# QData/ChromeGCN

Hardware: AMD Instinct MI355X
Metric: GCN windows/sec (2-layer, d_model=128) on GM12878 Hi-C graph (higher is better)
Workload: dtype f32

## Files before the change

### chromegcn_amd/_lib.py

```python
import ctypes
import os

import torch

from . import _build

_c_int = ctypes.c_int
_c_vp = ctypes.c_void_p
_c_sz = ctypes.c_size_t
_c_float = ctypes.c_float
_c_uint = ctypes.c_uint

_TYPES = {"i": _c_int, "u": _c_uint, "ll": ctypes.c_longlong, "z": _c_sz, "f": _c_float, "zp": ctypes.POINTER(_c_sz)}
_HEADER = {
    "cgcn_abi_version": (_c_int, ""),
    "cgcn_strerror": (ctypes.c_char_p, "code:i"),
    "cgcn_spmm": (_c_int, "stream n_rows:i n_cols:i S:i d:i rowptr col val row_scale X Y aux"),
    "cgcn_layer_fwd": (_c_int, "stream n:i S:i d:i rowptr col val row_scale X W b wg cg Xn Z H gate dropout_p:f rng_state "
                               "stream_id:u H_in colstats colstats_rows:i aux"),
    "cgcn_layer_fwd_colstats_plan": (_c_int, "n:i S:i d:i mode:i rows_per_tile"),
    "cgcn_debug_set_fwd_split_bytes": (None, "bytes:ll"),
    "cgcn_debug_set_products": (None, "mode:i"),
    "cgcn_debug_get_products": (_c_int, ""),
    "cgcn_debug_layer_fwd_route": (_c_int, "n:i S:i d:i aux colstats_rows:i"),
    "cgcn_debug_layer_bwd_route": (_c_int, "n:i S:i d:i"),
    "cgcn_layer_bwd_workspace_bytes": (_c_sz, "n:i S:i d:i"),
    "cgcn_layer_bwd": (_c_int, "stream n:i S:i d:i rowptr_t col_t val_t row_scale X Z H gate W wg dXn dgate dX dHs dW db dwg "
                               "dcg accumulate:i in_dropout_p:f rng_state in_stream_id:u head workspace workspace_bytes:z "
                               "aux_stream sgd aux_t"),
    "cgcn_debug_layer_bwd_phases": (_c_int, "stream n:i S:i d:i rowptr_t col_t val_t row_scale X Z H gate W wg dXn dgate dX dHs "
                                            "dW db dwg dcg accumulate:i in_dropout_p:f rng_state in_stream_id:u head workspace "
                                            "workspace_bytes:z phases:i aux_t"),
    "cgcn_layer_bwd_co": (_c_int, "stream n:i S:i d:i rowptr_t col_t val_t row_scale X Z H gate W wg dXn dgate dX dHs dW db "
                                  "dwg dcg accumulate:i in_dropout_p:f rng_state in_stream_id:u head workspace "
                                  "workspace_bytes:z aux_stream sgd aux_t companion"),
    "cgcn_debug_layer_bwd_co_route": (_c_int, "n:i S:i d:i rowptr_t col_t val_t have_dX:i aux_t companion"),
    "cgcn_head_workspace_bytes": (_c_sz, "n:i S:i d:i C:i"),
    "cgcn_head_workspace_layout": (_c_int, "n:i S:i d:i C:i dym_offset:zp bnc_offset:zp part_offset:zp"),
    "cgcn_head_bwd_partials": (_c_int, "n:i"),
    "cgcn_head_fwd": (_c_int, "stream n:i S:i d:i C:i X bn_w bn_b run_mean run_var num_batches_tracked momentum:f eps:f "
                              "training:i W_out b_out target dropout_p:f rng_state probs loss dpred save_mean save_invstd "
                              "workspace workspace_bytes:z"),
    "cgcn_head_logits": (_c_int, "stream n:i S:i d:i C:i X bn_w bn_b run_mean run_var eps:f W_out b_out logits"),
    "cgcn_head_train": (_c_int, "stream n:i S:i d:i C:i X bn_w bn_b run_mean run_var num_batches_tracked momentum:f eps:f "
                                "W_out b_out target dropout_p:f rng_state probs loss save_mean save_invstd col_stats "
                                "col_stats_tiles:i col_stats_rows:i workspace workspace_bytes:z"),
    "cgcn_debug_head_train_phases": (_c_int, "stream n:i S:i d:i C:i X bn_w bn_b run_mean run_var num_batches_tracked "
                                             "momentum:f eps:f W_out b_out target dropout_p:f rng_state probs loss save_mean "
                                             "save_invstd col_stats col_stats_tiles:i col_stats_rows:i workspace "
                                             "workspace_bytes:z phases:i"),
    "cgcn_head_bwd": (_c_int, "stream n:i S:i d:i C:i X bn_w bn_b save_mean save_invstd W_out dpred dloss dropout_p:f "
                              "rng_state dX dW_out db_out dbn_w dbn_b accumulate:i workspace workspace_bytes:z"),
    "cgcn_sddmm": (_c_int, "stream n:i S:i d:i rowptr col A B out accumulate:i"),
    "cgcn_saliency_normalize": (_c_int, "stream n:i rowptr val raw out"),
    "cgcn_graph_count": (_c_int, "stream n:i adj_type:i rowptr_in col_in val_in row_counts rowptr_out"),
    "cgcn_graph_fill": (_c_int, "stream n:i adj_type:i rowptr_in col_in val_in rowptr_out col_out val_out row_scale "
                                "symmetric_flag"),
    "cgcn_metrics_workspace_bytes": (_c_sz, "n:ll C:i"),
    "cgcn_multilabel_metrics": (_c_int, "stream n:ll C:i probs targets fdr_cutoff:f out workspace workspace_bytes:z"),
    "cgcn_multilabel_metrics_nonneg": (_c_int, "stream n:ll C:i probs targets fdr_cutoff:f out bad workspace "
                                               "workspace_bytes:z"),
    "cgcn_sgd_step": (_c_int, "stream count:ll param grad momentum_buf lr:f momentum:f weight_decay:f nesterov:i "
                              "grad_scale:f rng_state"),
    "cgcn_adam_step": (_c_int, "stream count:ll param grad exp_avg exp_avg_sq step n_step:i ticket lr:f beta1:f beta2:f "
                               "eps:f weight_decay:f grad_scale:f rng_state"),
    "cgcn_ablation_prepare": (_c_int, "stream n:i C:i targets label_bits pos_lists pos_ranks pos_counts"),
    "cgcn_ablation_workspace_bytes": (_c_sz, "n_inst:i S:i d:i layers:i"),
    "cgcn_ablation_layer": (_c_int, "stream n:i S:i d:i rowptr col val row_scale X X_inst W b wg cg label_bits C:i pos_list "
                                    "pos_rank n_pos:i cols n_cols:i X_out removed"),
    "cgcn_ablation_head": (_c_int, "stream n:i S:i d:i C:i X X_inst bn_w bn_b run_mean run_var eps:f W_out b_out pos_lists "
                                   "pos_counts label:i n_pos:i cols n_cols:i removed base M"),
    "cgcn_ablation_mask": (_c_int, "stream n:i C:i rowptr col val row_scale label_bits label_i:i label_j:i val_out "
                                   "row_scale_out removed"),
    "cgcn_ablation_reduce": (_c_int, "stream n:i S:i C:i logits pos_lists pos_counts label:i col_label:i removed base M"),
    "cgcn_hic_workspace_bytes": (_c_sz, "M:ll N:i capacity:ll K:ll"),
    "cgcn_hic_count": (_c_int, "stream M:ll pos1 pos2 window_start N:i workspace workspace_bytes:z n_survivors"),
    "cgcn_hic_build": (_c_int, "stream M:ll pos1 pos2 count norm n_bins:ll resolution_bp:i window_start N:i K:ll capacity:ll "
                               "workspace workspace_bytes:z rowptr_out col_out nnz_out n_survivors"),
    "cgcn_hic_up_workspace_bytes": (_c_sz, "M:ll N:i capacity:ll K:ll resolution_bp:i window_bp:i n_window_bins:ll"),
    "cgcn_hic_count_up": (_c_int, "stream M:ll pos1 pos2 window_start N:i resolution_bp:i window_bp:i n_window_bins:ll workspace "
                                  "workspace_bytes:z n_survivors"),
    "cgcn_hic_build_up": (_c_int, "stream M:ll pos1 pos2 count norm n_bins:ll resolution_bp:i window_bp:i n_window_bins:ll "
                                  "window_start N:i K:ll capacity:ll workspace workspace_bytes:z rowptr_out col_out nnz_out "
                                  "n_survivors"),
    "cgcn_hic_count_dist": (_c_int, "stream M:ll pos1 pos2 window_start N:i min_distance_bp:ll workspace workspace_bytes:z "
                                    "n_survivors"),
    "cgcn_hic_build_dist": (_c_int, "stream M:ll pos1 pos2 count norm n_bins:ll resolution_bp:i window_start N:i K:ll "
                                    "capacity:ll min_distance_bp:ll expected n_expected:ll workspace workspace_bytes:z rowptr_out "
                                    "col_out nnz_out n_survivors"),
    "cgcn_hic_count_up_dist": (_c_int, "stream M:ll pos1 pos2 window_start N:i resolution_bp:i window_bp:i n_window_bins:ll "
                                       "min_distance_bp:ll workspace workspace_bytes:z n_survivors"),
    "cgcn_hic_build_up_dist": (_c_int, "stream M:ll pos1 pos2 count norm n_bins:ll resolution_bp:i window_bp:i n_window_bins:ll "
                                       "window_start N:i K:ll capacity:ll min_distance_bp:ll expected n_expected:ll workspace "
                                       "workspace_bytes:z rowptr_out col_out nnz_out n_survivors"),
    "cgcn_hicdist_workspace_bytes": (_c_sz, "M:ll n_bins:ll"),
    "cgcn_hicdist_sums": (_c_int, "stream M:ll pos1 pos2 count norm n_norm:ll resolution_bp:i n_bins:ll workspace "
                                  "workspace_bytes:z raw_out act_out sizes"),
    "cgcn_text_workspace_bytes": (_c_sz, "n_bytes:ll"),
    "cgcn_text_count": (_c_int, "stream text n_bytes:ll workspace workspace_bytes:z n_records"),
    "cgcn_text_parse": (_c_int, "stream text n_bytes:ll M:ll pos1_out pos2_out count_out flags flag_capacity:ll flag_totals "
                                "workspace workspace_bytes:z"),
    "cgcn_tsne_workspace_bytes": (_c_sz, "n:i"),
    "cgcn_tsne_sqdist": (_c_int, "stream n:i d:i ld:i X D"),
    "cgcn_tsne_affinities": (_c_int, "stream n:i ld:i D perplexity:f C beta"),
    "cgcn_tsne_symmetrize": (_c_int, "stream n:i ld:i C P workspace workspace_bytes:z"),
    "cgcn_tsne_gradient": (_c_int, "stream n:i ld:i P Y exaggeration:f grad want_kl:i workspace workspace_bytes:z"),
# ... 187 lines not shown
```

### chromegcn_amd/csrc/cgcn_head.hip

```cpp
#include "cgcn_common.hpp"

#define HEAD_STAT_BLOCKS 128
#define HEAD_TILE 16
#define HEADB_TILE 32
#ifndef HEAD_MAX_PARTIALS
#define HEAD_MAX_PARTIALS 256
#endif


template <int D>
__global__ __launch_bounds__(256) void k_head_colstats(int n, int S, int rows_per_blk, const float* __restrict__ X,
                                                       float* __restrict__ part) {
  constexpr int RL = 256 / D;
  __shared__ float sm[2][256];
  const int c = threadIdx.x % D, rl = threadIdx.x / D;
  const int r0 = blockIdx.x * rows_per_blk, r1 = min(n, r0 + rows_per_blk);
  for (int s = 0; s < S; ++s) {
    const float* Xs = X + (size_t)s * n * D + c;
    const float pivot = r0 < n ? fmaxf(Xs[(size_t)r0 * D], 0.f) : 0.f;
    float s1 = 0.f, s2 = 0.f;
    int i = r0 + rl;
    for (; i + 3 * RL < r1; i += 4 * RL) {
      float v[4];
#pragma unroll
      for (int u = 0; u < 4; ++u) v[u] = Xs[(size_t)(i + u * RL) * D];
#pragma unroll
      for (int u = 0; u < 4; ++u) {
        const float dlt = fmaxf(v[u], 0.f) - pivot;
        s1 += dlt;
        s2 += dlt * dlt;
      }
    }
    for (; i < r1; i += RL) {
      const float dlt = fmaxf(Xs[(size_t)i * D], 0.f) - pivot;
      s1 += dlt;
      s2 += dlt * dlt;
    }
    if (RL > 1) {
      if (rl > 0) { sm[0][threadIdx.x] = s1; sm[1][threadIdx.x] = s2; }
      __syncthreads();
      if (rl == 0) {
        for (int o = 1; o < RL; ++o) { s1 += sm[0][o * D + c]; s2 += sm[1][o * D + c]; }
      }
      __syncthreads();
    }
    if (rl == 0) {
      const float k = (float)max(r1 - r0, 1);
      float* p = part + (((size_t)blockIdx.x * S + s) * D + c) * 2;
      p[0] = pivot + s1 / k;
      p[1] = fmaxf(s2 - s1 * s1 / k, 0.f);
    }
  }
}

__device__ __forceinline__ void chan_combine_d(double& nA, double& meanA, double& m2A, double nB, double meanB, double m2B) {
  const double nAB = nA + nB;
  if (nAB > 0.0) {
    const double delta = meanB - meanA;
    meanA += delta * (nB / nAB);
    m2A += m2B + delta * delta * (nA * nB / nAB);
    nA = nAB;
  }
}

template <int COLS>
__global__ __launch_bounds__(1024) void k_head_bn_finalize(int n, int S, int D, int nblk, int rows_per_blk,
                                                           const float* __restrict__ part, float momentum, float eps,
                                                           float* __restrict__ run_mean, float* __restrict__ run_var,
                                                           long long* __restrict__ nbt, float* __restrict__ save_mean,
                                                           float* __restrict__ save_invstd) {
  constexpr int NSL = 1024 / COLS;
  constexpr int SPW = 64 / COLS;
  constexpr int NWV = 16;
  static_assert(COLS * SPW == 64 && NSL == SPW * NWV, "thread layout");
  constexpr int KEEP = 16;
  __shared__ double sm[2][NWV][COLS + 1];
  __shared__ double stat[2][COLS + 1];
  const int cl = threadIdx.x % COLS, slice = threadIdx.x / COLS, wave = threadIdx.x >> 6;
  const int CPB = COLS / S;
  const int s = cl / CPB, c = blockIdx.x * CPB + cl % CPB;
  if (blockIdx.x == 0 && threadIdx.x == 0 && nbt) nbt[0] += S;
  float rm = 0.f, rv = 0.f;
// ... 1263 lines not shown
#pragma unroll
              for (int s = 0; s < 2; ++s) {
                float dy = g * invS;
                if (DROP) dy = dropout_keep(key, (uint32_t)((s * n + i) * D + c), thresh) ? dy * keep_scale : 0.f;
                if (s == 1) dy = S2 ? dy : 0.f;
                const float xh = (fmaxf(xq[s][mb][e], 0.f) - mu[s]) * is[s];
                sdy[s] += dy;
                sdyx[s] += dy * xh;
              }
            }
          }
      }
      RS_STAMP(3);
      __syncthreads();
      RS_STAMP(4);
      if (k < mt) load_xq((int)blockIdx.x + k * G);
      if (k >= 1) {
        OPAQUE_LANE(r, q, lq);
        __builtin_amdgcn_s_setprio(0);
        const float* __restrict__ Pa = Pt[(k - 1) & 1] + q * LDP + r;
        const float* __restrict__ Ya = Yt[(k - 1) & 1] + q * LDY + own * 16 + r;
        float a0[NB], a1[NB], b0, b1;
        b0 = Ya[0];
#pragma unroll
        for (int ib = 0; ib < NB; ++ib) a0[ib] = Pa[ib * 16];
#pragma unroll
        for (int kk = 0; kk < TR / 4; kk += 2) {
          b1 = Ya[(kk + 1) * 4 * LDY];
#pragma unroll
          for (int ib = 0; ib < NB; ++ib) a1[ib] = Pa[(kk + 1) * 4 * LDP + ib * 16];
          __builtin_amdgcn_sched_barrier(0);
#pragma unroll
          for (int ib = 0; ib < NB; ++ib) accW[ib] = __builtin_amdgcn_mfma_f32_16x16x4f32(a0[ib], b0, accW[ib], 0, 0, 0);
          __builtin_amdgcn_sched_barrier(0);
          if (kk + 2 < TR / 4) {
            b0 = Ya[(kk + 2) * 4 * LDY];
#pragma unroll
            for (int ib = 0; ib < NB; ++ib) a0[ib] = Pa[(kk + 2) * 4 * LDP + ib * 16];
          }
          __builtin_amdgcn_sched_barrier(0);
#pragma unroll
          for (int ib = 0; ib < NB; ++ib) accW[ib] = __builtin_amdgcn_mfma_f32_16x16x4f32(a1[ib], b1, accW[ib], 0, 0, 0);
          __builtin_amdgcn_sched_barrier(0);
        }
        __builtin_amdgcn_s_setprio(0);
      }
      RS_STAMP(5);
      __syncthreads();
    }
    const int r = lane & 15, q = lane >> 4;
#pragma unroll
    for (int ib = 0; ib < CBMAX; ++ib)
#pragma unroll
      for (int e = 0; e < 4; ++e) {
        const float v = ib < NB ? accW[ib < NB ? ib : 0][e] : 0.f;
        if (c0 + ib * 16 < CPT) P[(size_t)(c0 + ib * 16 + q * 4 + e) * D + own * 16 + r] = v;
      }
    if (last) {
      double* out = (double*)(P + CPT * D + CPT);
#pragma unroll
      for (int s = 0; s < 2; ++s) {
        double a = (double)sdy[s], b = (double)sdyx[s];
        a += __shfl_xor(a, 16); a += __shfl_xor(a, 32);
        b += __shfl_xor(b, 16); b += __shfl_xor(b, 32);
        if (q == 0) {
          out[s * D + own * 16 + r] = a;
          out[(2 + s) * D + own * 16 + r] = b;
          if (sa.acc && s < S) {
            int fa, fb;
            head_bacc_points(wmax, 16, keep_scale, n, fa, fb);
            unsigned long long* bb = bacc_base(sa.acc, S, D);
            bacc_add(bb, S, D, (int)blockIdx.x & (STAT_ACC_SLOTS - 1), s, own * 16 + r, a, b, fa, fb);
            if (blockIdx.x == 0 && s == 0 && own == 0 && r == 0)
              bb[(size_t)STAT_ACC_SLOTS * S * D * 2 + BACC_EXP] = ((unsigned long long)(unsigned)(fb + 1024) << 32) | (unsigned long long)(unsigned)(fa + 1024);
          }
        }
      }
    }
    __syncthreads();
  }
#undef OPAQUE_LANE
}

template <bool MULTI, int NB, bool DROP>
__global__ __launch_bounds__(1024) void k_head_fused_sp(int n, int S, int C, const float* __restrict__ X,
                                                        const float* __restrict__ bn_w, const float* __restrict__ bn_b,
                                                        const float* __restrict__ mean, const float* __restrict__ invstd,
                                                        const float* __restrict__ Wout, const float* __restrict__ bout,
                                                        const float* __restrict__ target, float keep_scale, uint32_t thresh,
                                                        const unsigned long long* __restrict__ rng_state, float inv_count,
                                                        float* __restrict__ probs, float* __restrict__ loss_part,
                                                        float* __restrict__ dym, float* __restrict__ part,
                                                        int c0, int Cp, int CPT, int first_, int last_, HeadStatAcc sa) {
  constexpr int D = 128, TR = 16, EPL = 2, RPW = TR / 8;
  constexpr int LVT = TR * 256;
  constexpr int WLV = 128 * 256;
  __shared__ __attribute__((aligned(16))) unsigned char Wl[3 * WLV];
  __shared__ __attribute__((aligned(16))) unsigned char Ytb[2][3 * LVT];
  __shared__ __attribute__((aligned(16))) unsigned char Ptb[2][3 * LVT];
  __shared__ float lsum[8];
  __shared__ float wmax[16];
  const bool first = MULTI ? first_ != 0 : true, last = MULTI ? last_ != 0 : true;

  const int lane = threadIdx.x & 63;
  const int wave = __builtin_amdgcn_readfirstlane(threadIdx.x >> 6);
  const int own = wave & 7;
  const uint32_t key = DROP ? dropout_key(rng_state, HEAD_STREAM_ID) : 0u;
  const float invS = 1.f / (float)S;
  const bool S2 = S > 1;
  const int PS = head_part_stride(CPT, D);
  const int ntiles = (n + TR - 1) / TR;
  const int G = (int)gridDim.x;
  const int mt = (int)blockIdx.x < ntiles ? (ntiles - 1 - (int)blockIdx.x) / G + 1 : 0;
  float* P = part + (size_t)blockIdx.x * PS;

  float mwl = 0.f;
  for (int idx = threadIdx.x; idx < 128 * (D / 4); idx += 1024) {
    const int j = idx / (D / 4), c4 = idx % (D / 4);
    f32x4 v = (f32x4){0.f, 0.f, 0.f, 0.f};
    if (j < Cp) v = *(const f32x4*)&Wout[(size_t)(c0 + j) * D + c4 * 4];
    u32x2 h2, m2, l2;
    sp_split4(v, h2, m2, l2);
    unsigned char* w = Wl + j * 256 + (((c4 >> 1) ^ sp_sigma(j & 15)) << 4) + ((c4 & 1) << 3);
    *(u32x2*)w = h2;
    *(u32x2*)(w + WLV) = m2;
    *(u32x2*)(w + 2 * WLV) = l2;
    mwl = fmaxf(fmaxf(mwl, fmaxf(fabsf(v[0]), fabsf(v[1]))), fmaxf(fabsf(v[2]), fabsf(v[3])));
  }
  if (sa.acc && last) {
    float mw;
    if (MULTI) mw = head_wout_absmax(Wout, C * (D / 4), 1024);
    else {
      mw = mwl;
#pragma unroll
      for (int o = 32; o > 0; o >>= 1) mw = fmaxf(mw, __shfl_xor(mw, o, WAVE));
    }
    if ((threadIdx.x & 63) == 0) wmax[threadIdx.x >> 6] = mw;
  }
  float* const stash = (float*)Ptb[1];
  static_assert(3 * LVT >= 6 * D * (int)sizeof(float), "the stash fits a P tile");
  if (sa.acc) head_stat_stage<D>(sa, n, S, stash, 1024);
#define OPAQUE_LANE(r_, q_, l_)          \
  int l_ = lane;                         \
  asm volatile("" : "+v"(l_));           \
  const int r_ = l_ & 15, q_ = l_ >> 4

  if (wave < 8) {
    float xv[RPW][2][EPL], tgv[4], mu[2][EPL], is[2][EPL], gw[EPL], gb[EPL];
    float dbo = 0.f, lacc = 0.f;
    const float bj = own * 16 + (lane & 15) < Cp ? bout[c0 + own * 16 + (lane & 15)] : 0.f;
#pragma unroll
    for (int e = 0; e < EPL; ++e) {
      const int c = lane * EPL + e;
      gw[e] = bn_w[c];
      gb[e] = bn_b[c];
    }
    bf16x8 wh[4], wm[4], wl[4];
    {
      const int r = lane & 15, q = lane >> 4;
      const int j = own * 16 + r;
#pragma unroll
      for (int s4 = 0; s4 < 4; ++s4) {
        f32x4 v0 = {0.f, 0.f, 0.f, 0.f}, v1 = v0;
        if (j < Cp) {
          v0 = *(const f32x4*)&Wout[(size_t)(c0 + j) * D + 32 * s4 + 8 * q];
          v1 = *(const f32x4*)&Wout[(size_t)(c0 + j) * D + 32 * s4 + 8 * q + 4];
        }
        const float v[8] = {v0[0], v0[1], v0[2], v0[3], v1[0], v1[1], v1[2], v1[3]};
        sp_split8(v, wh[s4], wm[s4], wl[s4]);
      }
    }
    auto load_rows = [&](int tile) {
      const int node0 = tile * TR;
#pragma unroll
      for (int t = 0; t < RPW; ++t) {
        const int i = node0 + own + t * 8;
#pragma unroll
        for (int s = 0; s < 2; ++s) {
          if (i < n && s < S) ld_row<EPL>(xv[t][s], &X[(unsigned)((s * n + i) * D + lane * EPL)]);
          else zero_row<EPL>(xv[t][s]);
        }
      }
    };
    auto load_targets = [&](int tile) {
      const int node0 = tile * TR;
      const int j = own * 16 + (lane & 15), q = lane >> 4;
#pragma unroll
      for (int e = 0; e < 4; ++e) {
        const int i = node0 + q * 4 + e;
        tgv[e] = (i < n && j < Cp) ? target[(unsigned)(i * C + c0 + j)] : 0.f;
      }
    };
    if (mt > 0) {
      load_rows(blockIdx.x);
      load_targets(blockIdx.x);
    }
    __syncthreads();
#pragma unroll
    for (int e = 0; e < EPL; ++e)
#pragma unroll
      for (int s = 0; s < 2; ++s) head_stat<D>(sa, stash, mean, invstd, s < S ? s : 0, lane * EPL + e, mu[s][e], is[s][e]);
    for (int k = 0; k <= mt; ++k) {
      const int tile = (int)blockIdx.x + k * G;
      const int node0 = tile * TR;
      if (k < mt) {
        int lane_ = lane;
        asm volatile("" : "+v"(lane_));
        unsigned char* __restrict__ Yb = Ytb[k & 1];
#pragma unroll
        for (int t = 0; t < RPW; ++t) {
          const int rr = own + t * 8;
          const int i = node0 + rr;
          float ym[EPL];
#pragma unroll
          for (int e = 0; e < EPL; ++e) {
            float y[2];
#pragma unroll
            for (int s = 0; s < 2; ++s) {
              y[s] = (fmaxf(xv[t][s][e], 0.f) - mu[s][e]) * is[s][e] * gw[e] + gb[e];
              if (DROP) y[s] = dropout_keep(key, (uint32_t)((s * n + i) * D + lane_ * EPL + e), thresh) ? y[s] * keep_scale : 0.f;
            }
            const float a = y[0] + (S2 ? y[1] : 0.f);
            ym[e] = i < n ? a * invS : 0.f;
          }
          uint32_t yh, ymid, yl;
          sp_split2(ym[0], ym[1], yh, ymid, yl);
          unsigned char* w = Yb + rr * 256 + (((lane_ >> 2) ^ sp_sigma(rr)) << 4) + ((lane_ & 3) << 2);
          *(uint32_t*)w = yh;
          *(uint32_t*)(w + LVT) = ymid;
          *(uint32_t*)(w + 2 * LVT) = yl;
        }
      }
      __syncthreads();
      f32x4 acc = {0.f, 0.f, 0.f, 0.f};
      if (k < mt) {
        if (k + 1 < mt) load_rows(tile + G);
        if (own < NB) {
          OPAQUE_LANE(r, q, lq);
          const unsigned char* __restrict__ Ya = Ytb[k & 1] + r * 256 + ((q ^ (sp_sigma(r) & 3)) << 4);
          const int hi = sp_sigma(r) >> 2;
          SpAcc sacc;
          sacc.zero();
#pragma unroll
          for (int s4 = 0; s4 < 4; ++s4) {
            const int o = (s4 ^ hi) << 6;
            const bf16x8 ah = __builtin_bit_cast(bf16x8, *(const u32x4*)(Ya + o));
            const bf16x8 am = __builtin_bit_cast(bf16x8, *(const u32x4*)(Ya + LVT + o));
            const bf16x8 al = __builtin_bit_cast(bf16x8, *(const u32x4*)(Ya + 2 * LVT + o));
            sacc.step(ah, am, al, wh[s4], wm[s4], wl[s4]);
          }
          acc = sacc.sum();
        }
      }
      if (k < mt) {
        unsigned char* __restrict__ Pb = Ptb[k & 1];
        OPAQUE_LANE(r, q, lq);
        const int j = own * 16 + r;
#pragma unroll
        for (int e = 0; e < 4; ++e) {
          const int row = q * 4 + e;
          const int i = node0 + row;
          const bool ok = i < n && j < Cp;
          const float pred = acc[e] + bj;
          const float en = __expf(-fabsf(pred));
          const float inv = __builtin_amdgcn_rcpf(1.f + en);
          const float p = pred >= 0.f ? inv : en * inv;
          const float l = fmaxf(pred, 0.f) - pred * tgv[e] + __logf(1.f + en);
          lacc += ok ? l : 0.f;
          if (ok) probs[(unsigned)(i * C + c0 + j)] = p;
          const float dp = ok ? (p - tgv[e]) * inv_count : 0.f;
          dbo += dp;
          uint16_t dh, dm, dl;
          sp_split1(dp, dh, dm, dl);
          unsigned char* w = Pb + row * 256 + (((j >> 3) ^ sp_sigma(row)) << 4) + ((j & 7) << 1);
          *(uint16_t*)w = dh;
          *(uint16_t*)(w + LVT) = dm;
          *(uint16_t*)(w + 2 * LVT) = dl;
        }
        if (k + 1 < mt) load_targets(tile + G);
      }
      __syncthreads();
    }
    dbo += __shfl_xor(dbo, 16);
    dbo += __shfl_xor(dbo, 32);
    if ((lane >> 4) == 0 && c0 + own * 16 + (lane & 15) < CPT) P[CPT * D + c0 + own * 16 + (lane & 15)] = dbo;
    lacc = wave_sum(lacc);
    if (lane == 0) lsum[own] = lacc;
    __syncthreads();
    if (threadIdx.x == 0) {
      float t = 0.f;
#pragma unroll
      for (int w = 0; w < 8; ++w) t += lsum[w];
      const float tl = first ? t : loss_part[blockIdx.x] + t;
      loss_part[blockIdx.x] = tl;
      if (sa.acc && last) head_loss_ticket(sa, S, D, tl, inv_count);
    }
  } else {
    f32x16 accW[2];
#pragma unroll
    for (int bb = 0; bb < 2; ++bb)
#pragma unroll
      for (int e = 0; e < 16; ++e) accW[bb][e] = 0.f;
    float sdy[2] = {0.f, 0.f}, sdyx[2] = {0.f, 0.f}, mu[2], is[2];
    __syncthreads();
    if (sa.acc && blockIdx.x == 0 && first && wave == 8) head_stat_bookkeeping<D>(sa, stash, S, lane);
#pragma unroll
    for (int s = 0; s < 2; ++s) head_stat<D>(sa, stash, mean, invstd, s < S ? s : 0, own * 16 + (lane & 15), mu[s], is[s]);
    float xq[2][4];
    auto load_xq = [&](int tile) {
      OPAQUE_LANE(r, q, lq);
      const int node0 = tile * TR, c = own * 16 + r;
#pragma unroll
      for (int s = 0; s < 2; ++s)
#pragma unroll
        for (int e = 0; e < 4; ++e) {
          const int i = node0 + q * 4 + e;
          xq[s][e] = (last && i < n && s < S) ? X[(unsigned)((s * n + i) * D + c)] : 0.f;
        }
    };
    for (int k = 0; k <= mt; ++k) {
      const int node0 = ((int)blockIdx.x + (k - 1) * G) * TR;
      f32x4 accY = {0.f, 0.f, 0.f, 0.f};
      if (k >= 1) {
        const unsigned char* __restrict__ Pb = Ptb[(k - 1) & 1];
        OPAQUE_LANE(r, q, lq);
        const unsigned char* __restrict__ Pa = Pb + r * 256 + ((q ^ (sp_sigma(r) & 3)) << 4);
        const int hi = sp_sigma(r) >> 2;
        const int qp = r >> 2, pp = r & 3;
        SpAcc2 sacc;
        sacc.zero();
#pragma unroll
        for (int s4 = 0; s4 < 4; ++s4) {
          const int o = (s4 ^ hi) << 6;
          const bf16x8 ah = __builtin_bit_cast(bf16x8, *(const u32x4*)(Pa + o));
          const bf16x8 am = __builtin_bit_cast(bf16x8, *(const u32x4*)(Pa + LVT + o));
          const bf16x8 al = __builtin_bit_cast(bf16x8, *(const u32x4*)(Pa + 2 * LVT + o));
          int wo[2];
#pragma unroll
          for (int rd = 0; rd < 2; ++rd) {
            const int lrow = 32 * s4 + 8 * q + 4 * rd + qp;
            wo[rd] = lrow * 256 + (((2 * own + (pp >> 1)) ^ sp_sigma(lrow & 15)) << 4) + ((pp & 1) << 3);
          }
          const bf16x8 bh = tr_pair(Wl + wo[0], Wl + wo[1]);
          const bf16x8 bm = tr_pair(Wl + WLV + wo[0], Wl + WLV + wo[1]);
          const bf16x8 bl = tr_pair(Wl + 2 * WLV + wo[0], Wl + 2 * WLV + wo[1]);
          sacc.step(ah, am, al, bh, bm, bl);
        }
        accY = sacc.sum();
        if (MULTI && !first) {
          const int c = own * 16 + r;
#pragma unroll
          for (int e = 0; e < 4; ++e) {
            const int i = node0 + q * 4 + e;
            accY[e] += i < n ? dym[(unsigned)(i * D + c)] : 0.f;
          }
        }
      }
      if (k >= 1) {
        OPAQUE_LANE(r, q, lq);
        const int c = own * 16 + r;
#pragma unroll
        for (int e = 0; e < 4; ++e) {
          const int i = node0 + q * 4 + e;
          const float g = accY[e];
          if (i < n) dym[(unsigned)(i * D + c)] = g;
          if (last) {
#pragma unroll
            for (int s = 0; s < 2; ++s) {
              float dy = g * invS;
              if (DROP) dy = dropout_keep(key, (uint32_t)((s * n + i) * D + c), thresh) ? dy * keep_scale : 0.f;
              if (s == 1) dy = S2 ? dy : 0.f;
              const float xh = (fmaxf(xq[s][e], 0.f) - mu[s]) * is[s];
              sdy[s] += dy;
              sdyx[s] += dy * xh;
            }
          }
        }
      }
      __syncthreads();
      if (k < mt) load_xq((int)blockIdx.x + k * G);
      if (k >= 1) {
        int lq = lane;
        asm volatile("" : "+v"(lq));
        const int hh = lq >> 5, c16 = (lq >> 4) & 1, qp = (lq & 15) >> 2, pp = lq & 3;
        const int cbk = own >> 1, lb0 = 2 * (own & 1);
        const unsigned char* __restrict__ Pb = Ptb[(k - 1) & 1];
        const unsigned char* __restrict__ Yb = Ytb[(k - 1) & 1];
        int ty[2], tp[2];
#pragma unroll
        for (int rd = 0; rd < 2; ++rd) {
          const int row = 8 * hh + 4 * rd + qp, sg = sp_sigma(row);
          ty[rd] = row * 256 + (((4 * cbk + 2 * c16 + (pp >> 1)) ^ sg) << 4) + ((pp & 1) << 3);
          tp[rd] = row * 256 + (((4 * lb0 + 2 * c16 + (pp >> 1)) ^ sg) << 4) + ((pp & 1) << 3);
        }
        bf16x8 yf[3];
#pragma unroll
        for (int v = 0; v < 3; ++v) yf[v] = tr_pair(Yb + v * LVT + ty[0], Yb + v * LVT + ty[1]);
#pragma unroll
        for (int bb = 0; bb < 2; ++bb) {
          bf16x8 pf[3];
#pragma unroll
          for (int v = 0; v < 3; ++v) pf[v] = tr_pair(Pb + v * LVT + (tp[0] ^ (bb << 6)), Pb + v * LVT + (tp[1] ^ (bb << 6)));
          accW[bb] = __builtin_amdgcn_mfma_f32_32x32x16_bf16(pf[2], yf[0], accW[bb], 0, 0, 0);
          accW[bb] = __builtin_amdgcn_mfma_f32_32x32x16_bf16(pf[0], yf[2], accW[bb], 0, 0, 0);
          accW[bb] = __builtin_amdgcn_mfma_f32_32x32x16_bf16(pf[1], yf[1], accW[bb], 0, 0, 0);
          accW[bb] = __builtin_amdgcn_mfma_f32_32x32x16_bf16(pf[1], yf[0], accW[bb], 0, 0, 0);
          accW[bb] = __builtin_amdgcn_mfma_f32_32x32x16_bf16(pf[0], yf[1], accW[bb], 0, 0, 0);
          accW[bb] = __builtin_amdgcn_mfma_f32_32x32x16_bf16(pf[0], yf[0], accW[bb], 0, 0, 0);
        }
      }
      __syncthreads();
    }
    {
      const int hh = lane >> 5, cbk = own >> 1, lb0 = 2 * (own & 1);
#pragma unroll
      for (int bb = 0; bb < 2; ++bb)
#pragma unroll
        for (int e = 0; e < 16; ++e) {
          const int lab = 32 * (lb0 + bb) + (e & 3) + 8 * (e >> 2) + 4 * hh;
          if (c0 + (lab & ~15) < CPT) P[(size_t)(c0 + lab) * D + 32 * cbk + (lane & 31)] = accW[bb][e];
        }
    }
    const int r = lane & 15, q = lane >> 4;
    if (last) {
      double* out = (double*)(P + CPT * D + CPT);
#pragma unroll
      for (int s = 0; s < 2; ++s) {
        double a = (double)sdy[s], b = (double)sdyx[s];
        a += __shfl_xor(a, 16); a += __shfl_xor(a, 32);
        b += __shfl_xor(b, 16); b += __shfl_xor(b, 32);
        if (q == 0) {
          out[s * D + own * 16 + r] = a;
          out[(2 + s) * D + own * 16 + r] = b;
          if (sa.acc && s < S) {
            int fa, fb;
            head_bacc_points(wmax, 16, keep_scale, n, fa, fb);
            unsigned long long* bb = bacc_base(sa.acc, S, D);
            bacc_add(bb, S, D, (int)blockIdx.x & (STAT_ACC_SLOTS - 1), s, own * 16 + r, a, b, fa, fb);
            if (blockIdx.x == 0 && s == 0 && own == 0 && r == 0)
              bb[(size_t)STAT_ACC_SLOTS * S * D * 2 + BACC_EXP] = ((unsigned long long)(unsigned)(fb + 1024) << 32) | (unsigned long long)(unsigned)(fa + 1024);
          }
        }
      }
    }
    __syncthreads();
  }
#undef OPAQUE_LANE
}

__global__ __launch_bounds__(512) void k_head_bwd_finalize(int wslab0, int wslabs, int P, int n, int S, int D, int C, int CP,
                                                           const float* __restrict__ part, float* __restrict__ dWout,
                                                           float* __restrict__ dbout, float* __restrict__ dbn_w,
                                                           float* __restrict__ dbn_b, float* __restrict__ bnc,
                                                           int accumulate, const float* __restrict__ dloss) {
  if ((int)blockIdx.x < wslabs)
    head_finalize_slab<512>(wslab0 + blockIdx.x, P, D, C, CP, part, dWout, dbout, accumulate, dloss);
// ... 99 lines not shown
  return CGCN_OK;
}

int cgcn_head_bwd_partials(int n) { return head_bwd_partials(n); }

size_t cgcn_head_workspace_bytes(int n, int S, int d, int C) {
  if (head_check(n, S, d, C) != CGCN_OK) return 0;
  return 4 * (align4(ws_stats(S, d)) + align4(ws_loss(n)) + align4(ws_dym(n, d)) + align4(ws_bnc(d)) + align4(ws_part(n, d, C)));
}

int cgcn_head_fwd(cgcn_stream_t stream, int n, int S, int d, int C, const float* X, const float* bn_w,
                  const float* bn_b, float* run_mean, float* run_var, long long* num_batches_tracked, float momentum,
                  float eps, int training, const float* Wout, const float* bout, const float* target, float dropout_p,
                  const unsigned long long* rng_state, float* probs, float* loss, float* dpred, float* save_mean,
                  float* save_invstd, void* workspace, size_t workspace_bytes) {
  int rc = head_check(n, S, d, C);
  if (rc) return rc;
  if (!X || !bn_w || !bn_b || !Wout || !bout || !target || !probs || !loss || !workspace) return CGCN_ERR_BAD_ARG;
  if (!run_mean || !run_var) return CGCN_ERR_BAD_ARG;
  if (training && (!save_mean || !save_invstd || n < 2)) return CGCN_ERR_BAD_ARG;
  const bool drop = training && dropout_p > 0.f;
  if (drop && (!rng_state || dropout_p >= 1.f)) return CGCN_ERR_BAD_ARG;
  if (workspace_bytes < cgcn_head_workspace_bytes(n, S, d, C)) return CGCN_ERR_WORKSPACE;
  if (misaligned16(Wout) || misaligned16(workspace) || misaligned16(X)) return CGCN_ERR_BAD_ARG;
  hipStream_t st = (hipStream_t)stream;
  float* w_stats = (float*)workspace;
  float* w_loss = w_stats + align4(ws_stats(S, d));
  if (n == 0) {
    hipLaunchKernelGGL(k_sum_scale, dim3(1), dim3(256), 0, st, 0, w_loss, 0.f, loss);
    return launch_status();
  }
  if (training) {
    int rpb;
    const int nblk = head_stat_blocks(n, &rpb);
    if (d == 128) hipLaunchKernelGGL((k_head_colstats<128>), dim3(nblk), dim3(256), 0, st, n, S, rpb, X, w_stats);
    else hipLaunchKernelGGL((k_head_colstats<256>), dim3(nblk), dim3(256), 0, st, n, S, rpb, X, w_stats);
    if ((rc = launch_status())) return rc;
    launch_bn_finalize(st, n, S, d, nblk, rpb, w_stats, momentum, eps, run_mean, run_var, num_batches_tracked, save_mean, save_invstd);
    if ((rc = launch_status())) return rc;
  }
  const int blocks = (n + HEAD_TILE - 1) / HEAD_TILE;
  const float keep_scale = drop ? 1.f / (1.f - dropout_p) : 1.f;
  const uint32_t thresh = drop ? dropout_threshold(dropout_p) : 0u;
  const float inv_count = 1.f / ((float)n * (float)C);
  const float* mean = training ? save_mean : run_mean;
  const float* vr = training ? save_invstd : run_var;
#define HF(D_, NC_)                                                                                                   \
  hipLaunchKernelGGL((k_head_fwd<D_, NC_>), dim3(blocks), dim3(512), 0, st, n, S, C, X, bn_w, bn_b, mean, vr,         \
                     training ? 0 : 1, eps, Wout, bout, target, keep_scale, thresh, rng_state, inv_count, probs,      \
                     training ? dpred : nullptr, w_loss, nullptr)
  if (d == 128) { if (C <= 128) HF(128, 1); else HF(128, 2); }
  else { if (C <= 128) HF(256, 1); else HF(256, 2); }
#undef HF
  if ((rc = launch_status())) return rc;
  hipLaunchKernelGGL(k_sum_scale, dim3(1), dim3(256), 0, st, blocks, w_loss, inv_count, loss);
  return launch_status();
}

int cgcn_head_logits(cgcn_stream_t stream, int n, int S, int d, int C, const float* X, const float* bn_w,
                     const float* bn_b, const float* run_mean, const float* run_var, float eps, const float* Wout,
                     const float* bout, float* logits) {
  int rc = head_check(n, S, d, C);
  if (rc) return rc;
  if (!X || !bn_w || !bn_b || !run_mean || !run_var || !Wout || !bout || !logits) return CGCN_ERR_BAD_ARG;
  if (misaligned16(Wout) || misaligned16(X)) return CGCN_ERR_BAD_ARG;
  if (n == 0) return CGCN_OK;
  hipStream_t st = (hipStream_t)stream;
  const int blocks = (n + HEAD_TILE - 1) / HEAD_TILE;
  for (int s = 0; s < S; ++s) {
    const float* Xs = X + (size_t)s * n * d;
    float* Ls = logits + (size_t)s * n * C;
#define HF(D_, NC_)                                                                                                   \
  hipLaunchKernelGGL((k_head_fwd<D_, NC_>), dim3(blocks), dim3(512), 0, st, n, 1, C, Xs, bn_w, bn_b, run_mean, run_var, \
                     1, eps, Wout, bout, nullptr, 1.f, 0u, nullptr, 0.f, nullptr, nullptr, nullptr, Ls)
    if (d == 128) { if (C <= 128) HF(128, 1); else HF(128, 2); }
    else { if (C <= 128) HF(256, 1); else HF(256, 2); }
#undef HF
    if ((rc = launch_status())) return rc;
  }
  return CGCN_OK;
}

}

static int head_train_impl(cgcn_stream_t stream, int n, int S, int d, int C, const float* X, const float* bn_w,
                    const float* bn_b, float* run_mean, float* run_var, long long* num_batches_tracked, float momentum,
                    float eps, const float* Wout, const float* bout, const float* target, float dropout_p,
                    const unsigned long long* rng_state, float* probs, float* loss, float* save_mean, float* save_invstd,
                    const float* col_stats, int col_stats_tiles, int col_stats_rows, void* workspace,
                    size_t workspace_bytes, int phases) {
  int rc = head_check(n, S, d, C);
  if (rc) return rc;
  if (!X || !bn_w || !bn_b || !Wout || !bout || !target || !probs || !loss || !workspace || !run_mean || !run_var ||
      !save_mean || !save_invstd || n < 2)
    return CGCN_ERR_BAD_ARG;
  const size_t acc_tile_bytes = (size_t)S * d * 2 * sizeof(float);
  const bool stat_acc = col_stats && col_stats_rows == -1;
  if (stat_acc && ((size_t)col_stats_tiles * acc_tile_bytes < stat_acc_words(S, d) * 8 || ((uintptr_t)col_stats & 7)))
    return CGCN_ERR_BAD_ARG;
  if (col_stats && !stat_acc && (col_stats_rows < 1 || col_stats_tiles != (n + col_stats_rows - 1) / col_stats_rows)) return CGCN_ERR_BAD_ARG;
  const bool drop = dropout_p > 0.f;
  if (drop && (!rng_state || dropout_p >= 1.f)) return CGCN_ERR_BAD_ARG;
  if (workspace_bytes < cgcn_head_workspace_bytes(n, S, d, C)) return CGCN_ERR_WORKSPACE;
  if (misaligned16(Wout) || misaligned16(workspace) || misaligned16(X)) return CGCN_ERR_BAD_ARG;
  hipStream_t st = (hipStream_t)stream;
  float* w_stats = (float*)workspace;
  float* w_loss = w_stats + align4(ws_stats(S, d));
  float* w_dym = w_loss + align4(ws_loss(n));
  float* w_bnc = w_dym + align4(ws_dym(n, d));
  float* w_part = w_bnc + align4(ws_bnc(d));
  int rpb;
  int nblk = head_stat_blocks(n, &rpb);
  const float* stats = w_stats;
  if (col_stats) {
    stats = col_stats;
    nblk = col_stats_tiles;
    rpb = col_stats_rows;
  } else if (phases & 1) {
    if (d == 128) hipLaunchKernelGGL((k_head_colstats<128>), dim3(nblk), dim3(256), 0, st, n, S, rpb, X, w_stats);
    else hipLaunchKernelGGL((k_head_colstats<256>), dim3(nblk), dim3(256), 0, st, n, S, rpb, X, w_stats);
    if ((rc = launch_status())) return rc;
  }
  if ((phases & 1) && !stat_acc) {
    launch_bn_finalize(st, n, S, d, nblk, rpb, stats, momentum, eps, run_mean, run_var, num_batches_tracked, save_mean, save_invstd);
    if ((rc = launch_status())) return rc;
  }
  const HeadStatAcc sa = {stat_acc ? (const unsigned long long*)col_stats : nullptr, eps, momentum,
                          run_mean, run_var, (phases & 1) ? num_batches_tracked : nullptr, save_mean, save_invstd, loss};
  const HeadStatAcc sa_prof = {sa.acc, eps, 0.f, run_mean, run_var, nullptr, save_mean, save_invstd, loss};
  const int P = head_bwd_partials(n);
  const int CP = head_cp(C);
  const float keep_scale = drop ? 1.f / (1.f - dropout_p) : 1.f;
  const uint32_t thresh = drop ? dropout_threshold(dropout_p) : 0u;
  const float inv_count = 1.f / ((float)n * (float)C);
  for (int c0 = 0; c0 < C && (phases & 2); c0 += 128) {
    const int Cp = C - c0 < 128 ? C - c0 : 128;
    const int first = c0 == 0, last = c0 + 128 >= C;
#define HFU(D_)                                                                                                        \
    hipLaunchKernelGGL((k_head_fused<D_, 8>), dim3(P), dim3(512), 0, st, n, S, C, X, bn_w, bn_b, save_mean, save_invstd, \
                       Wout, bout, target, keep_scale, thresh, rng_state, inv_count, probs, w_loss, w_dym, w_part, c0, Cp, \
                       CP, first, last, (phases & 1) ? sa : sa_prof)
    if (d == 128 && HEAD_RS) {
      const bool nb7 = Cp > 96 && Cp <= 112;
#ifndef HEAD_TR16_COST_PCT
#define HEAD_TR16_COST_PCT 55
#endif
      auto periods = [&](int tr) { return (((n + tr - 1) / tr) + P - 1) / P + 1; };
      const bool tr16 = HEAD_TR16_COST_PCT > 0 && periods(16) * HEAD_TR16_COST_PCT < periods(32) * 100;
#define HRS2(M_, NB_, DR_, NRB_)                                                                                       \
        hipLaunchKernelGGL((k_head_fused_rs<M_, NB_, DR_, NRB_>), dim3(P), dim3(1024), 0, st, n, S, C, X, bn_w, bn_b, save_mean, save_invstd, \
                         Wout, bout, target, keep_scale, thresh, rng_state, inv_count, probs, w_loss, w_dym, w_part, c0, Cp, \
                         CP, first, last, (phases & 1) ? sa : sa_prof)
#define HSP(M_, NB_, DR_)                                                                                              \
        hipLaunchKernelGGL((k_head_fused_sp<M_, NB_, DR_>), dim3(P), dim3(1024), 0, st, n, S, C, X, bn_w, bn_b, save_mean, save_invstd, \
                         Wout, bout, target, keep_scale, thresh, rng_state, inv_count, probs, w_loss, w_dym, w_part, c0, Cp, \
                         CP, first, last, (phases & 1) ? sa : sa_prof)
      const bool sph = cgcn_debug_get_products() != CGCN_PRODUCTS_FP32_CHAIN;
#define HRS(M_, NB_)                                                                                                   \
      do {                                                                                                             \
        if (sph) { if (thresh) HSP(M_, NB_, true); else HSP(M_, NB_, false); }                                          \
        else if (thresh) { if (tr16) HRS2(M_, NB_, true, 1); else HRS2(M_, NB_, true, 2); }                             \
        else { if (tr16) HRS2(M_, NB_, false, 1); else HRS2(M_, NB_, false, 2); }                                       \
      } while (0)
      if (C <= 128) { if (nb7) HRS(false, 7); else HRS(false, 8); }
      else { if (nb7) HRS(true, 7); else HRS(true, 8); }
#undef HRS
#undef HRS2
#undef HSP
    }
    else if (d == 128) HFU(128);
    else HFU(256);
#undef HFU
    if ((rc = launch_status())) return rc;
  }
  if (!(phases & 4) || stat_acc) return CGCN_OK;
  hipLaunchKernelGGL(k_head_train_finish, dim3(1 + d / HEAD_STAT_COLS), dim3(512), 0, st, P, n, S, d, CP, w_part, w_bnc,
                     w_loss, inv_count, loss);
  return launch_status();
}

extern "C" {

int cgcn_head_train(cgcn_stream_t stream, int n, int S, int d, int C, const float* X, const float* bn_w,
                    const float* bn_b, float* run_mean, float* run_var, long long* num_batches_tracked, float momentum,
                    float eps, const float* Wout, const float* bout, const float* target, float dropout_p,
                    const unsigned long long* rng_state, float* probs, float* loss, float* save_mean, float* save_invstd,
                    const float* col_stats, int col_stats_tiles, int col_stats_rows, void* workspace,
                    size_t workspace_bytes) {
  return head_train_impl(stream, n, S, d, C, X, bn_w, bn_b, run_mean, run_var, num_batches_tracked, momentum, eps, Wout, bout,
                         target, dropout_p, rng_state, probs, loss, save_mean, save_invstd, col_stats, col_stats_tiles,
                         col_stats_rows, workspace, workspace_bytes, 7);
}

int cgcn_debug_head_train_phases(cgcn_stream_t stream, int n, int S, int d, int C, const float* X, const float* bn_w,
                                 const float* bn_b, float* run_mean, float* run_var, long long* num_batches_tracked,
                                 float momentum, float eps, const float* Wout, const float* bout, const float* target,
                                 float dropout_p, const unsigned long long* rng_state, float* probs, float* loss,
                                 float* save_mean, float* save_invstd, const float* col_stats, int col_stats_tiles,
                                 int col_stats_rows, void* workspace, size_t workspace_bytes, int phases) {
  if (phases < 1 || phases > 7) return CGCN_ERR_BAD_ARG;
  return head_train_impl(stream, n, S, d, C, X, bn_w, bn_b, run_mean, run_var, num_batches_tracked, momentum, eps, Wout, bout,
                         target, dropout_p, rng_state, probs, loss, save_mean, save_invstd, col_stats, col_stats_tiles,
                         col_stats_rows, workspace, workspace_bytes, phases);
}

int cgcn_head_bwd(cgcn_stream_t stream, int n, int S, int d, int C, const float* X, const float* bn_w,
                  const float* bn_b, const float* save_mean, const float* save_invstd, const float* Wout,
                  const float* dpred, const float* dloss, float dropout_p, const unsigned long long* rng_state,
                  float* dX, float* dWout, float* dbout, float* dbn_w, float* dbn_b, int accumulate, void* workspace,
                  size_t workspace_bytes) {
  int rc = head_check(n, S, d, C);
  if (rc) return rc;
  if (!X || !bn_w || !bn_b || !save_mean || !save_invstd || !Wout || !dWout || !dbout || !dbn_w || !dbn_b || !workspace)
    return CGCN_ERR_BAD_ARG;
  const bool fused = dpred == nullptr;
  if (fused && dX) return CGCN_ERR_UNSUPPORTED;
  const bool drop = dropout_p > 0.f;
  if (drop && (!rng_state || dropout_p >= 1.f)) return CGCN_ERR_BAD_ARG;
  if (workspace_bytes < cgcn_head_workspace_bytes(n, S, d, C)) return CGCN_ERR_WORKSPACE;
  if (misaligned16(X) || (dX && misaligned16(dX)) || misaligned16(workspace) || n < 1) return CGCN_ERR_BAD_ARG;
  hipStream_t st = (hipStream_t)stream;
  float* w = (float*)workspace;
  float* w_dym = w + align4(ws_stats(S, d)) + align4(ws_loss(n));
  float* w_bnc = w_dym + align4(ws_dym(n, d));
  float* w_part = w_bnc + align4(ws_bnc(d));
  const int P = head_bwd_partials(n);
  const int CP = head_cp(C);
  const float keep_scale = drop ? 1.f / (1.f - dropout_p) : 1.f;
  const uint32_t thresh = drop ? dropout_threshold(dropout_p) : 0u;
  if (!fused) {
    for (int c0 = 0; c0 < C; c0 += 128) {
      const int Cp = C - c0 < 128 ? C - c0 : 128;
      const int first = c0 == 0, last = c0 + 128 >= C;
#define HB(D_)                                                                                                         \
      hipLaunchKernelGGL((k_head_bwd<D_, 8>), dim3(P), dim3(512), 0, st, n, S, C, X, bn_w, bn_b, save_mean, save_invstd, \
                         Wout, dpred, dloss, keep_scale, thresh, rng_state, w_dym, w_part, c0, Cp, CP, first, last)
      if (d == 128) HB(128); else HB(256);
#undef HB
      if ((rc = launch_status())) return rc;
    }
  }
  const float* fin_scale = fused ? dloss : nullptr;
  const int wslabs = (CP * d + CP) / 64, sblocks = d / HEAD_STAT_COLS;
  if (fused) {
    return CGCN_OK;
  }
  if (!dX) {
    hipLaunchKernelGGL(k_head_bwd_finalize, dim3(sblocks), dim3(512), 0, st, 0, 0, P, n, S, d, C, CP, w_part, dWout,
// ... 20 lines not shown
```

### include/chromegcn.h

```cpp
#ifndef CHROMEGCN_H
#define CHROMEGCN_H

#include <stddef.h>
#include <stdint.h>

#ifdef __cplusplus
extern "C" {
#endif

#define CGCN_OK 0
#define CGCN_ERR_BAD_ARG (-1)
#define CGCN_ERR_UNSUPPORTED (-2)
#define CGCN_ERR_LAUNCH (-3)
#define CGCN_ERR_WORKSPACE (-4)

#define CGCN_ABI_VERSION 26

typedef void *cgcn_stream_t;

typedef struct cgcn_graph_aux {
  const uint16_t *col16;
  const int32_t *row_order;
  int32_t max_row_len;
  int32_t band_halfwidth;
  const int32_t *bp_rowptr;
  const int32_t *bp_col;
  const uint16_t *bp_col16;
  const int32_t *bp_row_order;
} cgcn_graph_aux;

int cgcn_abi_version(void);

const char *cgcn_strerror(int code);

int cgcn_spmm(cgcn_stream_t stream, int n_rows, int n_cols, int S, int d,
              const int32_t *rowptr, const int32_t *col, const float *val, const float *row_scale,
              const float *X, float *Y, const cgcn_graph_aux *aux);

int cgcn_layer_fwd(cgcn_stream_t stream, int n, int S, int d,
                   const int32_t *rowptr, const int32_t *col, const float *val, const float *row_scale,
                   const float *X, const float *W, const float *b, const float *wg, const float *cg,
                   float *Xn, float *Z, float *H, float *gate,
                   float dropout_p, const unsigned long long *rng_state, unsigned int stream_id,
                   const float *H_in, float *colstats, int colstats_rows, const cgcn_graph_aux *aux);

#define CGCN_COLSTATS_RECORDS 0
#define CGCN_COLSTATS_ACCUMULATE 1
#define CGCN_COLSTATS_ROWS_ACCUMULATE (-1)
#define CGCN_COLSTATS_ROWS_ZERO_ONLY (-2)
#define CGCN_COLSTATS_ROWS_ACCUMULATE_ZEROED (-3)

int cgcn_layer_fwd_colstats_plan(int n, int S, int d, int mode, int *rows_per_tile);

void cgcn_debug_set_fwd_split_bytes(long long bytes);

#define CGCN_PRODUCTS_FP32_CHAIN 0
#define CGCN_PRODUCTS_SPLIT 1
void cgcn_debug_set_products(int mode);
int cgcn_debug_get_products(void);

int cgcn_debug_layer_fwd_route(int n, int S, int d, const cgcn_graph_aux *aux, int colstats_rows);
int cgcn_debug_layer_bwd_route(int n, int S, int d);

typedef struct cgcn_head_grad {
  const float *dym;
  const float *bnc;
  const float *save_mean;
  const float *save_invstd;
  const float *bn_w;
  float dropout_p;
  const unsigned long long *rng_state;
  const float *part;
  int n_partials;
  int C;
  float *dW_out;
  float *db_out;
  int accumulate;
  const float *dloss;
  float *dbn_w;
  float *dbn_b;
  const void *stat_acc;
} cgcn_head_grad;

typedef struct cgcn_sgd_fuse {
  float *param;
  const float *grad;
  float *momentum_buf;
  long long count;
  float lr, momentum, weight_decay, grad_scale;
  int nesterov;
  unsigned long long *rng_state;
} cgcn_sgd_fuse;

size_t cgcn_layer_bwd_workspace_bytes(int n, int S, int d);

int cgcn_layer_bwd(cgcn_stream_t stream, int n, int S, int d,
                   const int32_t *rowptr_t, const int32_t *col_t, const float *val_t, const float *row_scale,
                   const float *X, const float *Z, const float *H, const float *gate,
                   const float *W, const float *wg,
                   const float *dXn, const float *dgate,
                   float *dX, float *dHs, float *dW, float *db, float *dwg, float *dcg,
                   int accumulate, float in_dropout_p, const unsigned long long *rng_state,
                   unsigned int in_stream_id, const cgcn_head_grad *head,
                   void *workspace, size_t workspace_bytes, cgcn_stream_t aux_stream,
                   const cgcn_sgd_fuse *sgd, const cgcn_graph_aux *aux_t);

int cgcn_debug_layer_bwd_phases(cgcn_stream_t stream, int n, int S, int d,
                                const int32_t *rowptr_t, const int32_t *col_t, const float *val_t, const float *row_scale,
                                const float *X, const float *Z, const float *H, const float *gate,
                                const float *W, const float *wg, const float *dXn, const float *dgate,
                                float *dX, float *dHs, float *dW, float *db, float *dwg, float *dcg,
                                int accumulate, float in_dropout_p, const unsigned long long *rng_state,
                                unsigned int in_stream_id, const cgcn_head_grad *head,
                                void *workspace, size_t workspace_bytes, int phases, const cgcn_graph_aux *aux_t);

typedef struct cgcn_spmm_job {
  int n, S, d;
  const int32_t *rowptr;
  const int32_t *col;
  const float *val;
  const float *row_scale;
  const float *X;
  float *H;
  const cgcn_graph_aux *aux;
} cgcn_spmm_job;

int cgcn_layer_bwd_co(cgcn_stream_t stream, int n, int S, int d,
                      const int32_t *rowptr_t, const int32_t *col_t, const float *val_t, const float *row_scale,
                      const float *X, const float *Z, const float *H, const float *gate,
                      const float *W, const float *wg,
                      const float *dXn, const float *dgate,
                      float *dX, float *dHs, float *dW, float *db, float *dwg, float *dcg,
                      int accumulate, float in_dropout_p, const unsigned long long *rng_state,
                      unsigned int in_stream_id, const cgcn_head_grad *head,
                      void *workspace, size_t workspace_bytes, cgcn_stream_t aux_stream,
                      const cgcn_sgd_fuse *sgd, const cgcn_graph_aux *aux_t, const cgcn_spmm_job *companion);

int cgcn_debug_layer_bwd_co_route(int n, int S, int d, const int32_t *rowptr_t, const int32_t *col_t, const float *val_t,
                                  int have_dX, const cgcn_graph_aux *aux_t, const cgcn_spmm_job *companion);

size_t cgcn_head_workspace_bytes(int n, int S, int d, int C);

// ... 322 lines not shown
```

Measured before the change: 61.14 million.

## Keep head W_out split operands resident in registers instead of LDS

Adds a WREG variant of the fused split-precision head kernel, used when C<=128. Each wave loads its slice of W_out once, splits it into three bf16 parts held in registers, and feeds them straight to the matrix step. This removes the 96KB LDS copy of W_out and the per-tile LDS transposed reads. The cost is higher register pressure, an extra global load pass, and a changed absmax and fma ordering in the stat accumulation. The variant is on by default and can be switched back with an env var or a debug setter.

```diff
diff --git a/chromegcn_amd/_lib.py b/chromegcn_amd/_lib.py
--- a/chromegcn_amd/_lib.py
+++ b/chromegcn_amd/_lib.py
@@ -22,6 +22,8 @@
     "cgcn_debug_set_fwd_split_bytes": (None, "bytes:ll"),
     "cgcn_debug_set_products": (None, "mode:i"),
     "cgcn_debug_get_products": (_c_int, ""),
+    "cgcn_debug_set_head_wout": (None, "where:i"),
+    "cgcn_debug_get_head_wout": (_c_int, ""),
     "cgcn_debug_layer_fwd_route": (_c_int, "n:i S:i d:i aux colstats_rows:i"),
     "cgcn_debug_layer_bwd_route": (_c_int, "n:i S:i d:i"),
     "cgcn_layer_bwd_workspace_bytes": (_c_sz, "n:i S:i d:i"),
diff --git a/chromegcn_amd/csrc/cgcn_head.hip b/chromegcn_amd/csrc/cgcn_head.hip
--- a/chromegcn_amd/csrc/cgcn_head.hip
+++ b/chromegcn_amd/csrc/cgcn_head.hip
@@ -1,3 +1,6 @@
+#include <atomic>
+#include <cstdlib>
+
 #include "cgcn_common.hpp"
 
 #define HEAD_STAT_BLOCKS 128
@@ -1427,7 +1430,7 @@
 #undef OPAQUE_LANE
 }
 
-template <bool MULTI, int NB, bool DROP>
+template <bool MULTI, int NB, bool DROP, bool WREG = false>
 __global__ __launch_bounds__(1024) void k_head_fused_sp(int n, int S, int C, const float* __restrict__ X,
                                                         const float* __restrict__ bn_w, const float* __restrict__ bn_b,
                                                         const float* __restrict__ mean, const float* __restrict__ invstd,
@@ -1440,7 +1443,8 @@
   constexpr int D = 128, TR = 16, EPL = 2, RPW = TR / 8;
   constexpr int LVT = TR * 256;
   constexpr int WLV = 128 * 256;
-  __shared__ __attribute__((aligned(16))) unsigned char Wl[3 * WLV];
+  static_assert(!(WREG && MULTI), "resident W_out operands: one label pass");
+  __shared__ __attribute__((aligned(16))) unsigned char Wl[WREG ? 16 : 3 * WLV];
   __shared__ __attribute__((aligned(16))) unsigned char Ytb[2][3 * LVT];
   __shared__ __attribute__((aligned(16))) unsigned char Ptb[2][3 * LVT];
   __shared__ float lsum[8];
@@ -1460,7 +1464,7 @@
   float* P = part + (size_t)blockIdx.x * PS;
 
   float mwl = 0.f;
-  for (int idx = threadIdx.x; idx < 128 * (D / 4); idx += 1024) {
+  for (int idx = threadIdx.x; !WREG && idx < 128 * (D / 4); idx += 1024) {
     const int j = idx / (D / 4), c4 = idx % (D / 4);
     f32x4 v = (f32x4){0.f, 0.f, 0.f, 0.f};
     if (j < Cp) v = *(const f32x4*)&Wout[(size_t)(c0 + j) * D + c4 * 4];
@@ -1472,7 +1476,7 @@
     *(u32x2*)(w + 2 * WLV) = l2;
     mwl = fmaxf(fmaxf(mwl, fmaxf(fabsf(v[0]), fabsf(v[1]))), fmaxf(fabsf(v[2]), fabsf(v[3])));
   }
-  if (sa.acc && last) {
+  if (!WREG && sa.acc && last) {
     float mw;
     if (MULTI) mw = head_wout_absmax(Wout, C * (D / 4), 1024);
     else {
@@ -1513,7 +1517,16 @@
         }
         const float v[8] = {v0[0], v0[1], v0[2], v0[3], v1[0], v1[1], v1[2], v1[3]};
         sp_split8(v, wh[s4], wm[s4], wl[s4]);
-      }
+        if (WREG) {
+#pragma unroll
+          for (int e = 0; e < 8; ++e) mwl = fmaxf(mwl, fabsf(v[e]));
+        }
+      }
+    }
+    if (WREG && sa.acc) {
+#pragma unroll
+      for (int o = 32; o > 0; o >>= 1) mwl = fmaxf(mwl, __shfl_xor(mwl, o, WAVE));
+      if (lane == 0) wmax[wave] = mwl;
     }
     auto load_rows = [&](int tile) {
       const int node0 = tile * TR;
@@ -1647,6 +1660,19 @@
 #pragma unroll
       for (int e = 0; e < 16; ++e) accW[bb][e] = 0.f;
     float sdy[2] = {0.f, 0.f}, sdyx[2] = {0.f, 0.f}, mu[2], is[2];
+    bf16x8 qh[4], qm[4], ql[4];
+    float wraw[4][8];
+    if (WREG) {
+      const int r = lane & 15, q = lane >> 4;
+#pragma unroll
+      for (int s4 = 0; s4 < 4; ++s4)
+#pragma unroll
+        for (int e = 0; e < 8; ++e) {
+          const int j = 32 * s4 + 8 * q + e;
+          wraw[s4][e] = j < Cp ? Wout[(size_t)(c0 + j) * D + own * 16 + r] : 0.f;
+        }
+      if (sa.acc && lane == 0) wmax[wave] = 0.f;
+    }
     __syncthreads();
     if (sa.acc && blockIdx.x == 0 && first && wave == 8) head_stat_bookkeeping<D>(sa, stash, S, lane);
 #pragma unroll
@@ -1663,7 +1689,21 @@
           xq[s][e] = (last && i < n && s < S) ? X[(unsigned)((s * n + i) * D + c)] : 0.f;
         }
     };
-    for (int k = 0; k <= mt; ++k) {
+    if (WREG) {
+      __syncthreads();
+      if (0 < mt) load_xq((int)blockIdx.x);
+#pragma unroll
+      for (int s4 = 0; s4 < 4; ++s4) {
+        sp_split8(wraw[s4], qh[s4], qm[s4], ql[s4]);
+        u32x4 th = __builtin_bit_cast(u32x4, qh[s4]), tm = __builtin_bit_cast(u32x4, qm[s4]), tl = __builtin_bit_cast(u32x4, ql[s4]);
+        asm volatile("" : "+v"(th), "+v"(tm), "+v"(tl));
+        qh[s4] = __builtin_bit_cast(bf16x8, th);
+        qm[s4] = __builtin_bit_cast(bf16x8, tm);
+        ql[s4] = __builtin_bit_cast(bf16x8, tl);
+      }
+      __syncthreads();
+    }
+    for (int k = WREG ? 1 : 0; k <= mt; ++k) {
       const int node0 = ((int)blockIdx.x + (k - 1) * G) * TR;
       f32x4 accY = {0.f, 0.f, 0.f, 0.f};
       if (k >= 1) {
@@ -1686,6 +1726,10 @@
             const int lrow = 32 * s4 + 8 * q + 4 * rd + qp;
             wo[rd] = lrow * 256 + (((2 * own + (pp >> 1)) ^ sp_sigma(lrow & 15)) << 4) + ((pp & 1) << 3);
           }
+          if (WREG) {
+            sacc.step(ah, am, al, qh[s4], qm[s4], ql[s4]);
+            continue;
+          }
           const bf16x8 bh = tr_pair(Wl + wo[0], Wl + wo[1]);
           const bf16x8 bm = tr_pair(Wl + WLV + wo[0], Wl + WLV + wo[1]);
           const bf16x8 bl = tr_pair(Wl + 2 * WLV + wo[0], Wl + 2 * WLV + wo[1]);
@@ -1717,6 +1761,14 @@
               if (s == 1) dy = S2 ? dy : 0.f;
               const float xh = (fmaxf(xq[s][e], 0.f) - mu[s]) * is[s];
               sdy[s] += dy;
+              if (WREG) {
+                if (DROP && s == 1) {
+                  float t = dy * xh;
+                  asm volatile("" : "+v"(t));
+                  sdyx[s] += t;
+                } else sdyx[s] = __builtin_fmaf(dy, xh, sdyx[s]);
+                continue;
+              }
               sdyx[s] += dy * xh;
             }
           }
@@ -1982,6 +2034,21 @@
 }
 
 }
+
+#ifndef HEADSP_WOUT
+#define HEADSP_WOUT CGCN_HEAD_WOUT_REGISTERS
+#endif
+static int head_wout_default() {
+  const char* e = getenv("CGCN_HEAD_WOUT");
+  if (e && (e[0] == 'l' || e[0] == '0')) return CGCN_HEAD_WOUT_LDS;
+  if (e && (e[0] == 'r' || e[0] == '1')) return CGCN_HEAD_WOUT_REGISTERS;
+  return HEADSP_WOUT;
+}
+static std::atomic<int> g_head_wout{head_wout_default()};
+extern "C" void cgcn_debug_set_head_wout(int where) {
+  g_head_wout.store((where == CGCN_HEAD_WOUT_LDS || where == CGCN_HEAD_WOUT_REGISTERS) ? where : head_wout_default());
+}
+extern "C" int cgcn_debug_get_head_wout(void) { return g_head_wout.load(); }
 
 static int head_train_impl(cgcn_stream_t stream, int n, int S, int d, int C, const float* X, const float* bn_w,
                     const float* bn_b, float* run_mean, float* run_var, long long* num_batches_tracked, float momentum,
@@ -2056,14 +2123,24 @@
                          Wout, bout, target, keep_scale, thresh, rng_state, inv_count, probs, w_loss, w_dym, w_part, c0, Cp, \
                          CP, first, last, (phases & 1) ? sa : sa_prof)
       const bool sph = cgcn_debug_get_products() != CGCN_PRODUCTS_FP32_CHAIN;
+      const bool wreg = sph && C <= 128 && g_head_wout.load() == CGCN_HEAD_WOUT_REGISTERS;
+#define HSPW(NB_, DR_)                                                                                                 \
+        hipLaunchKernelGGL((k_head_fused_sp<false, NB_, DR_, true>), dim3(P), dim3(1024), 0, st, n, S, C, X, bn_w, bn_b, save_mean, save_invstd, \
+                         Wout, bout, target, keep_scale, thresh, rng_state, inv_count, probs, w_loss, w_dym, w_part, c0, Cp, \
+                         CP, first, last, (phases & 1) ? sa : sa_prof)
 #define HRS(M_, NB_)                                                                                                   \
       do {                                                                                                             \
         if (sph) { if (thresh) HSP(M_, NB_, true); else HSP(M_, NB_, false); }                                          \
         else if (thresh) { if (tr16) HRS2(M_, NB_, true, 1); else HRS2(M_, NB_, true, 2); }                             \
         else { if (tr16) HRS2(M_, NB_, false, 1); else HRS2(M_, NB_, false, 2); }                                       \
       } while (0)
-      if (C <= 128) { if (nb7) HRS(false, 7); else HRS(false, 8); }
+      if (wreg) {
+        if (nb7) { if (thresh) HSPW(7, true); else HSPW(7, false); }
+        else { if (thresh) HSPW(8, true); else HSPW(8, false); }
+      }
+      else if (C <= 128) { if (nb7) HRS(false, 7); else HRS(false, 8); }
       else { if (nb7) HRS(true, 7); else HRS(true, 8); }
+#undef HSPW
 #undef HRS
 #undef HRS2
 #undef HSP
diff --git a/include/chromegcn.h b/include/chromegcn.h
--- a/include/chromegcn.h
+++ b/include/chromegcn.h
@@ -58,6 +58,11 @@
 #define CGCN_PRODUCTS_SPLIT 1
 void cgcn_debug_set_products(int mode);
 int cgcn_debug_get_products(void);
+
+#define CGCN_HEAD_WOUT_LDS 0
+#define CGCN_HEAD_WOUT_REGISTERS 1
+void cgcn_debug_set_head_wout(int where);
+int cgcn_debug_get_head_wout(void);
 
 int cgcn_debug_layer_fwd_route(int n, int S, int d, const cgcn_graph_aux *aux, int colstats_rows);
 int cgcn_debug_layer_bwd_route(int n, int S, int d);
```

Result: faster. 62.12 million, median of 6 (+1.6%).
